# reazon-research/ReazonSpeech

Hardware: AMD Instinct MI355X
Metric: RTFx (audio-sec/wall-sec), FastConformer-RNNT 619M batch=256 (higher is better)
Workload: dtype bf16

## Files before the change

reazonspeech_amd/csrc/k_rnnt.hip:

```cpp
#include <cstdio>
#include <cstdlib>

#include "k_rnnt_common.h"

namespace {

__global__ void rnnt_init_kernel(DecodeState st, const int32_t* __restrict__ enc_lens, int B, int blank,
                                 int32_t* __restrict__ n_ids) {
    __shared__ int n_alive_s;
    if (threadIdx.x == 0) n_alive_s = 0;
    __syncthreads();
    for (int b = threadIdx.x; b < B; b += blockDim.x) {
        st.tcur[b] = 0; st.sym[b] = 0; st.token[b] = blank; st.act[b] = b;
        if (st.token2) st.token2[b] = -1;
        n_ids[b] = 0;
        if (enc_lens[b] > 0) st.alive[atomicAdd(&n_alive_s, 1)] = b;
    }
    __syncthreads();
    if (threadIdx.x == 0) { st.counters[0] = B; st.counters[1] = 0; st.counters[2] = n_alive_s; st.counters[3] = 0; }
}

__global__ __launch_bounds__(1024) void rnnt_lstm_kernel(DecodeState st, int layer, int B, int H,
                                                        const float* __restrict__ embed,
                                                        const float* __restrict__ W ,
// ... 215 lines not shown
        if (nblk >= 2) { compute(f0); f0 = f1; }
        compute(f0);
    }
#pragma unroll
    for (int ri = 0; ri < 2; ++ri)
#pragma unroll
        for (int cj = 0; cj < 4; ++cj)
#pragma unroll
            for (int r = 0; r < 4; ++r) part[wave][ri * 16 + 4 * kk + r][cj * 16 + li] = acc[ri][cj][r];
    __syncthreads();
    if (tid >= 256) { if (WALK) { __syncthreads(); continue; } return; }
    const int i = tid >> 3, c0 = (tid & 7) * 8;
    const bool row_ok = rt * 32 + i < n_rows;
    const int brow = rows_s[i];
    float best = -INFINITY;
    int best_idx = 0x7fffffff;
#pragma unroll
    for (int e = 0; e < 8; ++e) {
        const int v = ct * 64 + c0 + e;
        float s = part[0][i][c0 + e];
#pragma unroll
        for (int sl = 1; sl < SPLITK_TILE; ++sl) s = s + part[sl][i][c0 + e];
        if (v < N) {
            s = s + bias[v];
            if (MODE == 0) { if (row_ok) st.g[(size_t)brow * N + v] = s; }
            else if (!ARGMAX) { if (row_ok) st.zapprox[(size_t)brow * (64 * n_ctiles) + v] = s; }
            else if (s > best) { best = s; best_idx = v; }
        }
    }
    if (ARGMAX) {
#pragma unroll
        for (int off = 1; off < 8; off <<= 1) {
            const float ov = __shfl_xor(best, off, 64);
            const int oi = __shfl_xor(best_idx, off, 64);
            if (ov > best || (ov == best && oi < best_idx)) { best = ov; best_idx = oi; }
        }
        if ((tid & 7) == 0 && row_ok) {
            st.pmax[(size_t)brow * n_ctiles + ct] = best;
            st.pidx[(size_t)brow * n_ctiles + ct] = best_idx;
        }
    } else if (MODE == 0 && row_ok) {
        const int stride = gridDim.x * 64;
        for (int l = 0; l < L; ++l)
            for (int u = ct * 64 + c0; u < H; u += stride)
#pragma unroll
                for (int e = 0; e < 8; ++e) {
                    if (u + e >= H) break;
                    const size_t o = ((size_t)l * B + brow) * H + u + e;
                    st.h[o] = st.h_tmp[o];
                    st.c[o] = st.c_tmp[o];
                }
    }
    if (!WALK) return;
    __syncthreads();
    }
}

__global__ __launch_bounds__(256) void rnnt_finalize_kernel(DecodeState st, const int32_t* __restrict__ enc_lens,
                                                            int B, int n_ctiles, int blank, int max_symbols,
                                                            int u_max, int step, int32_t* __restrict__ ids,
                                                            int32_t* __restrict__ frames, int32_t* __restrict__ n_ids) {
    const int lane = threadIdx.x & 63;
    const int slot = blockIdx.x * 4 + (threadIdx.x >> 6);
    const int n_alive = st.counters[2 + (step & 1)];
    if (slot >= n_alive) return;
    const int b = st.alive[(size_t)(step & 1) * B + slot];
    float val = -INFINITY;
    int idx = 0x7fffffff;
    for (int ctile = lane; ctile < n_ctiles; ctile += 64) {
        const float ov = st.pmax[(size_t)b * n_ctiles + ctile];
        const int oi = st.pidx[(size_t)b * n_ctiles + ctile];
        if (ov > val || (ov == val && oi < idx)) { val = ov; idx = oi; }
    }
#pragma unroll
    for (int off = 32; off > 0; off >>= 1) {
        const float ov = __shfl_xor(val, off, 64);
        const int oi = __shfl_xor(idx, off, 64);
        if (ov > val || (ov == val && oi < idx)) { val = ov; idx = oi; }
    }
    if (lane != 0) return;
    int t = st.tcur[b], sy = st.sym[b];
    bool emitted = false;
    if (idx == blank || idx == st.unk || idx == 0x7fffffff) {
        t += 1; sy = 0;
    } else {
        const int n = n_ids[b];
        if (n < u_max) { ids[(size_t)b * u_max + n] = idx; frames[(size_t)b * u_max + n] = t; n_ids[b] = n + 1; }
        else st.counters[1] = 1;
        if (st.token2) st.token2[b] = st.token[b];
        st.token[b] = idx;
        emitted = true;
        sy += 1;
        if (sy >= max_symbols) { t += 1; sy = 0; }
    }
    st.tcur[b] = t; st.sym[b] = sy;
    if (t < enc_lens[b]) {
        const int pos = atomicAdd(&st.counters[2 + ((step + 1) & 1)], 1);
        st.alive[(size_t)((step + 1) & 1) * B + pos] = b;
        if (emitted) { const int pa = atomicAdd(&st.counters[0], 1); st.act[pa] = b; }
    }
}



__global__ __launch_bounds__(256) void rnnt_finalize_la_kernel(DecodeState st, const int32_t* __restrict__ enc_lens, int B, int n_ctiles,
                                                               int blank, int max_symbols, int u_max, int step, int la,
                                                               int32_t* __restrict__ ids, int32_t* __restrict__ frames,
                                                               int32_t* __restrict__ n_ids) {
    const int lane = threadIdx.x & 63;
    const int slot = blockIdx.x * 4 + (threadIdx.x >> 6);
    const int n_alive = st.counters[2 + (step & 1)];
    if (slot >= n_alive) return;
    const int b = st.alive[(size_t)(step & 1) * B + slot];
    const int T = enc_lens[b];
    int t = st.tcur[b], sy = st.sym[b];
    bool emitted = false;
    for (int j = 0; j < la && t < T; ++j) {
        float val = -INFINITY;
        int idx = 0x7fffffff;
        const size_t row = (size_t)b * la + j;
        for (int ctile = lane; ctile < n_ctiles; ctile += 64) {
            const float ov = st.pmax[row * n_ctiles + ctile];
            const int oi = st.pidx[row * n_ctiles + ctile];
            if (ov > val || (ov == val && oi < idx)) { val = ov; idx = oi; }
        }
#pragma unroll
        for (int off = 32; off > 0; off >>= 1) {
            const float ov = __shfl_xor(val, off, 64);
            const int oi = __shfl_xor(idx, off, 64);
            if (ov > val || (ov == val && oi < idx)) { val = ov; idx = oi; }
        }
        if (idx == blank || idx == st.unk || idx == 0x7fffffff) { t += 1; sy = 0; continue; }
        if (lane == 0) {
            const int n = n_ids[b];
            if (n < u_max) { ids[(size_t)b * u_max + n] = idx; frames[(size_t)b * u_max + n] = t; n_ids[b] = n + 1; }
            else st.counters[1] = 1;
            if (st.token2) st.token2[b] = st.token[b];
            st.token[b] = idx;
        }
        emitted = true;
        sy += 1;
        if (sy >= max_symbols) { t += 1; sy = 0; }
        break;
    }
    if (lane != 0) return;
    st.tcur[b] = t; st.sym[b] = sy;
    if (t < T) {
        const int pos = atomicAdd(&st.counters[2 + ((step + 1) & 1)], 1);
        st.alive[(size_t)((step + 1) & 1) * B + pos] = b;
        if (emitted) { const int pa = atomicAdd(&st.counters[0], 1); st.act[pa] = b; }
    }
}

__global__ __launch_bounds__(1024) void rnnt_lstm4_kernel(DecodeState st, int layer, int B, int H,
                                                         const float* __restrict__ embed,
                                                         const float* __restrict__ W4 ,
                                                         const float* __restrict__ bias ) {
    __shared__ float part[SPLITK_LSTM][32][17];
    __shared__ int rows_s[32];
    const int n_act = st.counters[0];
    const int rt = blockIdx.y, ug = blockIdx.x;
    if (rt * 32 >= n_act) return;
    const int tid = threadIdx.x, lane = tid & 63, wave = tid >> 6;
    if (tid < 32) {
        const int i = rt * 32 + tid;
        rows_s[tid] = st.act[i < n_act ? i : n_act - 1];
    }
    __syncthreads();
    const int li = lane & 15, kk = lane >> 4;
    const int lr = lane >> 2, lc = lane & 3;
    const int perm = 4 * (4 * li + kk);
    const int K = 2 * H, kslice = K / SPLITK_LSTM, nkb = K / 16;
    const float* xsrc[2];
    const float* hsrc[2];
#pragma unroll
    for (int ri = 0; ri < 2; ++ri) {
        const int row = rows_s[ri * 16 + lr];
        xsrc[ri] = layer == 0 ? embed + (size_t)st.token[row] * H : st.h_tmp + ((size_t)(layer - 1) * B + row) * H;
        hsrc[ri] = st.h + ((size_t)layer * B + row) * H;
    }
    const float* wfrag = W4 + ((size_t)ug * nkb) * 256 + lane * 4;
    f32x4_t acc[2] = {(f32x4_t){0.f, 0.f, 0.f, 0.f}, (f32x4_t){0.f, 0.f, 0.f, 0.f}};
    const int kbeg = wave * kslice, nblk = kslice / 16;
    float4 av[2][8], wv[8];
#pragma unroll
    for (int u = 0; u < 8; ++u)
        if (u < nblk) {
            const int k = kbeg + 16 * u + 4 * lc;
#pragma unroll
            for (int ri = 0; ri < 2; ++ri)
                av[ri][u] = (k < H) ? *reinterpret_cast<const float4*>(xsrc[ri] + k) : *reinterpret_cast<const float4*>(hsrc[ri] + (k - H));
            wv[u] = *reinterpret_cast<const float4*>(wfrag + (size_t)((kbeg >> 4) + u) * 256);
        }
#pragma unroll
    for (int u = 0; u < 8; ++u)
        if (u < nblk) {
            const float4 a0 = to_mfma_a_layout(av[0][u], perm), a1 = to_mfma_a_layout(av[1][u], perm);
#define RS_MFMA_E(c)                                                                         \
            acc[0] = __builtin_amdgcn_mfma_f32_16x16x4f32(a0.c, wv[u].c, acc[0], 0, 0, 0);   \
            acc[1] = __builtin_amdgcn_mfma_f32_16x16x4f32(a1.c, wv[u].c, acc[1], 0, 0, 0);
            RS_MFMA_E(x) RS_MFMA_E(y) RS_MFMA_E(z) RS_MFMA_E(w)
#undef RS_MFMA_E
        }
#pragma unroll
    for (int ri = 0; ri < 2; ++ri)
#pragma unroll
        for (int r = 0; r < 4; ++r) part[wave][ri * 16 + 4 * kk + r][li] = acc[ri][r];
    __syncthreads();
    if (tid >= 128) return;
    const int i = tid >> 2, u4 = tid & 3;
    if (rt * 32 + i >= n_act) return;
    const int brow = rows_s[i];
    const int unit = ug * 4 + u4;
    float z[4];
#pragma unroll
    for (int gt = 0; gt < 4; ++gt) {
        float sm = part[0][i][gt * 4 + u4];
#pragma unroll
        for (int sl = 1; sl < SPLITK_LSTM; ++sl) sm = sm + part[sl][i][gt * 4 + u4];
        z[gt] = sm + bias[gt * H + unit];
    }
    const float ig = rs_sigmoidf(z[0]), fg = rs_sigmoidf(z[1]), gg = rs_tanhf(z[2]), og = rs_sigmoidf(z[3]);
    const size_t o = ((size_t)layer * B + brow) * H + unit;
    const float cn = fmaf(fg, st.c[o], ig * gg);
    st.c_tmp[o] = cn;
    st.h_tmp[o] = og * rs_tanhf(cn);
}

__global__ __launch_bounds__(512) void rnnt_pred16_kernel(DecodeState st, int B, int L, int H, int N ,
                                                         const float* __restrict__ W, const float* __restrict__ bias) {
    __shared__ float part[SPLITK_TILE][32][17];
    __shared__ int rows_s[32];
    const int rt = blockIdx.y, ct = blockIdx.x;
    const int tid = threadIdx.x, lane = tid & 63, wave = tid >> 6;
    const int n_rows = st.counters[0];
    if (rt * 32 >= n_rows) return;
    if (tid < 32) {
        const int i = rt * 32 + tid;
        rows_s[tid] = st.act[i < n_rows ? i : n_rows - 1];
    }
    __syncthreads();
    const int li = lane & 15, kk = lane >> 4;
    const int lr = lane >> 2, lc = lane & 3;
    const int perm = 4 * (4 * li + kk);
    const int K = H, nkb = K / 16;
    const float* asrc[2];
#pragma unroll
    for (int ri = 0; ri < 2; ++ri) asrc[ri] = st.h_tmp + ((size_t)(L - 1) * B + rows_s[ri * 16 + lr]) * H;
    const float* wfrag = W + ((size_t)ct * nkb) * 256 + lane * 4;
    f32x4_t acc[2] = {(f32x4_t){0.f, 0.f, 0.f, 0.f}, (f32x4_t){0.f, 0.f, 0.f, 0.f}};
    const int kslice = K / SPLITK_TILE, kbeg = wave * kslice, nblk = kslice / 16;
    float4 av[2][8], wv[8];
#pragma unroll
    for (int u = 0; u < 8; ++u)
        if (u < nblk) {
            const int k = kbeg + 16 * u + 4 * lc;
#pragma unroll
            for (int ri = 0; ri < 2; ++ri) av[ri][u] = *reinterpret_cast<const float4*>(asrc[ri] + k);
            wv[u] = *reinterpret_cast<const float4*>(wfrag + (size_t)((kbeg >> 4) + u) * 256);
        }
#pragma unroll
    for (int u = 0; u < 8; ++u)
        if (u < nblk) {
            const float4 a0 = to_mfma_a_layout(av[0][u], perm), a1 = to_mfma_a_layout(av[1][u], perm);
#define RS_MFMA_E(c)                                                                         \
            acc[0] = __builtin_amdgcn_mfma_f32_16x16x4f32(a0.c, wv[u].c, acc[0], 0, 0, 0);   \
            acc[1] = __builtin_amdgcn_mfma_f32_16x16x4f32(a1.c, wv[u].c, acc[1], 0, 0, 0);
            RS_MFMA_E(x) RS_MFMA_E(y) RS_MFMA_E(z) RS_MFMA_E(w)
#undef RS_MFMA_E
        }
#pragma unroll
    for (int ri = 0; ri < 2; ++ri)
#pragma unroll
        for (int r = 0; r < 4; ++r) part[wave][ri * 16 + 4 * kk + r][li] = acc[ri][r];
    __syncthreads();
    const int i = tid >> 4, c = tid & 15;
    const bool row_ok = rt * 32 + i < n_rows;
    const int brow = rows_s[i];
    const int v = ct * 16 + c;
    if (row_ok && v < N) {
        float sm = part[0][i][c];
#pragma unroll
        for (int sl = 1; sl < SPLITK_TILE; ++sl) sm = sm + part[sl][i][c];
        st.g[(size_t)brow * N + v] = sm + bias[v];
    }
    if (row_ok) {
        const int nct = gridDim.x;
        for (int l = 0; l < L; ++l)
            for (int u = ct * 16 + c; u < H; u += nct * 16) {
                const size_t o = ((size_t)l * B + brow) * H + u;
                st.h[o] = st.h_tmp[o];
                st.c[o] = st.c_tmp[o];
            }
    }
}

__global__ __launch_bounds__(256) void rnnt_prep_kernel(DecodeState st, const float* __restrict__ f, int B, int Tp, int J,
                                                        int step) {
    const int lane = threadIdx.x & 63;
    const int slot = blockIdx.x * 4 + (threadIdx.x >> 6);
    if (blockIdx.x == 0 && threadIdx.x == 0) {
        st.counters[0] = 0;
        st.counters[2 + ((step + 1) & 1)] = 0;
    }
    if (slot >= st.counters[2 + (step & 1)]) return;
    const int b = st.alive[(size_t)(step & 1) * B + slot];
    int t = st.tcur[b];
    t = t < Tp ? t : Tp - 1;
    const float* fr = f + ((size_t)b * Tp + t) * J;
    const float* gr = st.g + (size_t)b * J;
    float ss = 0.0f;
    for (int k = 4 * lane; k < J; k += 256) {
        const float4 fv = *reinterpret_cast<const float4*>(fr + k), gv = *reinterpret_cast<const float4*>(gr + k);
        float a0, a1, a2, a3;
        if (st.joint_act) {
            a0 = rs_tanhf(fv.x + gv.x); a1 = rs_tanhf(fv.y + gv.y); a2 = rs_tanhf(fv.z + gv.z); a3 = rs_tanhf(fv.w + gv.w);
        } else {
            a0 = fmaxf(fv.x + gv.x, 0.0f); a1 = fmaxf(fv.y + gv.y, 0.0f); a2 = fmaxf(fv.z + gv.z, 0.0f); a3 = fmaxf(fv.w + gv.w, 0.0f);
        }
        ss = fmaf(a0, a0, fmaf(a1, a1, fmaf(a2, a2, fmaf(a3, a3, ss))));
        *reinterpret_cast<u16x4_t*>(st.a16 + (size_t)slot * J + k) = pack_bf16x4(a0, a1, a2, a3);
    }
    ss = wave_sum(ss);
    if (lane == 0) st.anorm[slot] = sqrtf(ss) * 1.0001f;
}

__global__ __launch_bounds__(256) void rnnt_screen_kernel(DecodeState st, const float* __restrict__ f, int B, int Tp, int J,
                                                          int Vpad, const uint16_t* __restrict__ W16,
                                                          const float* __restrict__ bpad, int step) {
    extern __shared__ __attribute__((aligned(16))) char scr_smem[];
    const int ldrow = J * 2 + 16;
    const int ct = blockIdx.x, rt = blockIdx.y;
    const int tid = threadIdx.x, lane = tid & 63, wave = tid >> 6;
    const int n_alive = st.counters[2 + (step & 1)];
    if (rt * 32 >= n_alive) return;
    const int col0 = (ct * 4 + wave) * 16;
    const bool has_cols = col0 < Vpad;
    const int li = lane & 15, kc = lane >> 4;
    const int nks = J / 32;
    const uint16_t* wrow = W16 + (size_t)((has_cols ? col0 : 0) + li) * J + kc * 8;
    bf16x8_t wf[20];
#pragma unroll
    for (int q = 0; q < 20; ++q)
        if (q < nks) wf[q] = *reinterpret_cast<const bf16x8_t*>(wrow + q * 32);
    const float bv = bpad[(has_cols ? col0 : 0) + li];
    {
        const int per_row = J / 8;
        for (int idx = tid; idx < 32 * per_row; idx += 256) {
            const int r = idx / per_row, c = idx - r * per_row;
            const int i = rt * 32 + r;
            const uint4 v = *reinterpret_cast<const uint4*>(st.a16 + (size_t)(i < n_alive ? i : n_alive - 1) * J + c * 8);
            *reinterpret_cast<uint4*>(scr_smem + r * ldrow + c * 16) = v;
        }
    }
    __syncthreads();
    if (!has_cols) return;
    f32x4_t acc[2] = {(f32x4_t){0.f, 0.f, 0.f, 0.f}, (f32x4_t){0.f, 0.f, 0.f, 0.f}};
#pragma unroll
    for (int q = 0; q < 20; ++q)
        if (q < nks) {
#pragma unroll
            for (int ri = 0; ri < 2; ++ri) {
                const bf16x8_t af = *reinterpret_cast<const bf16x8_t*>(scr_smem + (ri * 16 + li) * ldrow + (q * 32 + kc * 8) * 2);
                acc[ri] = __builtin_amdgcn_mfma_f32_16x16x32_bf16(af, wf[q], acc[ri], 0, 0, 0);
            }
        }
#pragma unroll
    for (int ri = 0; ri < 2; ++ri)
#pragma unroll
        for (int r = 0; r < 4; ++r) {
            const int slot = rt * 32 + ri * 16 + 4 * kc + r;
            if (slot < n_alive) st.zapprox[(size_t)slot * Vpad + col0 + li] = acc[ri][r] + bv;
        }
}

constexpr int VER_CAP = 1024;

__device__ __forceinline__ void verify_evaluate(const int* cand_s, int n_cand, const float* a_s, const float* __restrict__ Wrm,
                                                const float* __restrict__ bo, int J, int lane, float& best, int& best_idx) {
    const int cgrp = lane >> 3, sl = lane & 7;
    const int kslice = J / SPLITK_TILE, nblk = kslice / 16;
    for (int c0 = 0; c0 < n_cand; c0 += 8) {
        const bool valid = c0 + cgrp < n_cand;
        const int cand = valid ? cand_s[c0 + cgrp] : 0;
        const float* w = Wrm + (size_t)cand * J + sl * kslice;
        const float* as = a_s + sl * kslice;
        float4 wv[8][4];
#pragma unroll
        for (int u = 0; u < 8; ++u)
            if (u < nblk) {
#pragma unroll
                for (int kk = 0; kk < 4; ++kk) wv[u][kk] = *reinterpret_cast<const float4*>(w + 16 * u + 4 * kk);
            }
        float acc = 0.0f;
#pragma unroll
        for (int u = 0; u < 8; ++u)
            if (u < nblk) {
                float4 av[4];
#pragma unroll
                for (int kk = 0; kk < 4; ++kk) av[kk] = *reinterpret_cast<const float4*>(as + 16 * u + 4 * kk);
#define RS_CHAIN_E(cc) _Pragma("unroll") for (int kk = 0; kk < 4; ++kk) acc = fmaf(av[kk].cc, wv[u][kk].cc, acc);
                RS_CHAIN_E(x) RS_CHAIN_E(y) RS_CHAIN_E(z) RS_CHAIN_E(w)
#undef RS_CHAIN_E
            }
        float sum = __shfl(acc, lane & ~7, 64);
#pragma unroll
        for (int q = 1; q < SPLITK_TILE; ++q) sum = sum + __shfl(acc, (lane & ~7) + q, 64);
        float val = valid ? sum + bo[cand] : -INFINITY;
        int idx = valid ? cand : 0x7fffffff;
#pragma unroll
        for (int off = 8; off < 64; off <<= 1) {
            const float ov = __shfl_xor(val, off, 64);
            const int oi = __shfl_xor(idx, off, 64);
            if (ov > val || (ov == val && oi < idx)) { val = ov; idx = oi; }
        }
        if (val > best || (val == best && idx < best_idx)) { best = val; best_idx = idx; }
    }
}

__device__ __forceinline__ void verify_act_row(const DecodeState& st, const float* fr, const float* gr, float* a_s, int J, int tid, int nthr) {
    for (int k = 4 * tid; k < J; k += 4 * nthr) {
        const float4 fv = *reinterpret_cast<const float4*>(fr + k), gv = *reinterpret_cast<const float4*>(gr + k);
        if (st.joint_act)
            *reinterpret_cast<float4*>(a_s + k) = make_float4(rs_tanhf(fv.x + gv.x), rs_tanhf(fv.y + gv.y), rs_tanhf(fv.z + gv.z), rs_tanhf(fv.w + gv.w));
        else
            *reinterpret_cast<float4*>(a_s + k) = make_float4(fmaxf(fv.x + gv.x, 0.0f), fmaxf(fv.y + gv.y, 0.0f),
                                                              fmaxf(fv.z + gv.z, 0.0f), fmaxf(fv.w + gv.w, 0.0f));
    }
}

__device__ __forceinline__ void verify_commit(const DecodeState& st, int b, int t, int idx, const int32_t* __restrict__ enc_lens, int B,
                                              int blank, int max_symbols, int u_max, int step, int32_t* __restrict__ ids,
                                              int32_t* __restrict__ frames, int32_t* __restrict__ n_ids) {
    int sy = st.sym[b];
    bool emitted = false;
    if (idx == blank || idx == st.unk || idx == 0x7fffffff) {
        t += 1; sy = 0;
    } else {
        const int n = n_ids[b];
        if (n < u_max) { ids[(size_t)b * u_max + n] = idx; frames[(size_t)b * u_max + n] = t; n_ids[b] = n + 1; }
        else st.counters[1] = 1;
        if (st.token2) st.token2[b] = st.token[b];
        st.token[b] = idx;
        emitted = true;
        sy += 1;
        if (sy >= max_symbols) { t += 1; sy = 0; }
    }
    st.tcur[b] = t; st.sym[b] = sy;
    if (t < enc_lens[b]) {
        const int pos = atomicAdd(&st.counters[2 + ((step + 1) & 1)], 1);
        st.alive[(size_t)((step + 1) & 1) * B + pos] = b;
        if (emitted) { const int pa = atomicAdd(&st.counters[0], 1); st.act[pa] = b; }
    }
}

template <int NCH>
__global__ __launch_bounds__(256) void rnnt_verify_kernel(DecodeState st, const float* __restrict__ f,
                                                          const int32_t* __restrict__ enc_lens, int B, int Tp, int J, int V,
                                                          int Vpad, const float* __restrict__ Wrm ,
                                                          const float* __restrict__ bo, const float* __restrict__ wmax, int blank,
                                                          int max_symbols, int u_max, int step, int32_t* __restrict__ ids,
                                                          int32_t* __restrict__ frames, int32_t* __restrict__ n_ids) {
    extern __shared__ __attribute__((aligned(16))) char ver_smem[];
    constexpr int CAND_ROWS = NCH > 0 ? NCH * 64 : VER_CAP;
    const int lane = threadIdx.x & 63, wave = threadIdx.x >> 6;
    const int slot = blockIdx.x * 4 + wave;
    const int n_alive = st.counters[2 + (step & 1)];
    if (slot >= n_alive) return;
    const int b = st.alive[(size_t)(step & 1) * B + slot];
    const float* z = st.zapprox + (size_t)slot * Vpad;
    const int nchunk = (V + 63) / 64;
    float zr[NCH > 0 ? NCH : 1];
    float m = -INFINITY;
    if constexpr (NCH > 0) {
#pragma unroll
        for (int c = 0; c < NCH; ++c) zr[c] = (c * 64 + lane < V) ? z[c * 64 + lane] : -INFINITY;
#pragma unroll
        for (int c = 0; c < NCH; ++c) m = fmaxf(m, zr[c]);
    } else {
        for (int c = 0; c < nchunk; ++c) m = fmaxf(m, (c * 64 + lane < V) ? z[c * 64 + lane] : -INFINITY);
    }
    m = wave_max(m);
    const int t = st.tcur[b];
    const int tc = t < Tp ? t : Tp - 1;
    float* a_s = reinterpret_cast<float*>(ver_smem) + wave * J;
    verify_act_row(st, f + ((size_t)b * Tp + tc) * J, st.g + (size_t)b * J, a_s, J, lane, 64);
    const float thr = m - 0.01953125f * wmax[0] * st.anorm[slot];
    int* cand_s = reinterpret_cast<int*>(ver_smem + 4 * J * 4) + wave * CAND_ROWS;
    float best = -INFINITY;
    int best_idx = 0x7fffffff;
    int n_cand = 0;
    if constexpr (NCH > 0) {
#pragma unroll
        for (int c = 0; c < NCH; ++c) {
            const bool is = zr[c] >= thr;
            const unsigned long long mask = __ballot(is);
            if (is) cand_s[n_cand + __builtin_popcountll(mask & ((1ull << lane) - 1ull))] = c * 64 + lane;
            n_cand += __builtin_popcountll(mask);
        }
        __builtin_amdgcn_fence(__ATOMIC_ACQ_REL, "wavefront");
        __builtin_amdgcn_wave_barrier();
        verify_evaluate(cand_s, n_cand, a_s, Wrm, bo, J, lane, best, best_idx);
    } else {
        for (int c = 0; c < nchunk; ++c) {
            const bool is = c * 64 + lane < V && z[c * 64 + lane] >= thr;
            const unsigned long long mask = __ballot(is);
            if (is) cand_s[n_cand + __builtin_popcountll(mask & ((1ull << lane) - 1ull))] = c * 64 + lane;
            n_cand += __builtin_popcountll(mask);
            if (n_cand + 64 > VER_CAP || c == nchunk - 1) {
                __builtin_amdgcn_fence(__ATOMIC_ACQ_REL, "wavefront");
                __builtin_amdgcn_wave_barrier();
                verify_evaluate(cand_s, n_cand, a_s, Wrm, bo, J, lane, best, best_idx);
                __builtin_amdgcn_fence(__ATOMIC_ACQ_REL, "wavefront");
                __builtin_amdgcn_wave_barrier();
                n_cand = 0;
            }
        }
    }
    if (lane != 0) return;
    verify_commit(st, b, t, best_idx, enc_lens, B, blank, max_symbols, u_max, step, ids, frames, n_ids);
}

template <int NCHW>
__global__ __launch_bounds__(256) void rnnt_verify_wide_kernel(DecodeState st, const float* __restrict__ f,
                                                               const int32_t* __restrict__ enc_lens, int B, int Tp, int J, int V,
                                                               int Vpad, const float* __restrict__ Wrm ,
                                                               const float* __restrict__ bo, const float* __restrict__ wmax, int blank,
                                                               int max_symbols, int u_max, int step, int32_t* __restrict__ ids,
                                                               int32_t* __restrict__ frames, int32_t* __restrict__ n_ids) {
    extern __shared__ __attribute__((aligned(16))) char ver_smem[];
    const int lane = threadIdx.x & 63, wave = threadIdx.x >> 6;
    const int slot = blockIdx.x;
    const int n_alive = st.counters[2 + (step & 1)];
    if (slot >= n_alive) return;
    const int b = st.alive[(size_t)(step & 1) * B + slot];
    const float* z = st.zapprox + (size_t)slot * Vpad;
    float zr[NCHW];
#pragma unroll
    for (int c = 0; c < NCHW; ++c) {
        const int col = (wave * NCHW + c) * 64 + lane;
        zr[c] = col < V ? z[col] : -INFINITY;
    }
    float m = -INFINITY;
#pragma unroll
    for (int c = 0; c < NCHW; ++c) m = fmaxf(m, zr[c]);
    m = wave_max(m);
    float* a_s = reinterpret_cast<float*>(ver_smem);
    int* cand_s = reinterpret_cast<int*>(ver_smem + (size_t)J * 4) + wave * (NCHW * 64);
    float* red = reinterpret_cast<float*>(ver_smem + (size_t)J * 4 + (size_t)4 * NCHW * 64 * 4);
    const int t = st.tcur[b];
    const int tc = t < Tp ? t : Tp - 1;
    verify_act_row(st, f + ((size_t)b * Tp + tc) * J, st.g + (size_t)b * J, a_s, J, threadIdx.x, 256);
    if (lane == 0) red[wave] = m;
    __syncthreads();
    m = fmaxf(fmaxf(red[0], red[1]), fmaxf(red[2], red[3]));
    const float thr = m - 0.01953125f * wmax[0] * st.anorm[slot];
    int n_cand = 0;
#pragma unroll
    for (int c = 0; c < NCHW; ++c) {
        const bool is = zr[c] >= thr;
        const unsigned long long mask = __ballot(is);
        if (is) cand_s[n_cand + __builtin_popcountll(mask & ((1ull << lane) - 1ull))] = (wave * NCHW + c) * 64 + lane;
        n_cand += __builtin_popcountll(mask);
    }
    __builtin_amdgcn_fence(__ATOMIC_ACQ_REL, "wavefront");
    __builtin_amdgcn_wave_barrier();
    float best = -INFINITY;
    int best_idx = 0x7fffffff;
    verify_evaluate(cand_s, n_cand, a_s, Wrm, bo, J, lane, best, best_idx);
    if (lane == 0) { red[4 + wave] = best; reinterpret_cast<int*>(red)[8 + wave] = best_idx; }
    __syncthreads();
    if (threadIdx.x != 0) return;
#pragma unroll
    for (int w = 0; w < 4; ++w) {
        const float v = red[4 + w];
        const int i = reinterpret_cast<int*>(red)[8 + w];
        if (v > best || (v == best && i < best_idx)) { best = v; best_idx = i; }
    }
    verify_commit(st, b, t, best_idx, enc_lens, B, blank, max_symbols, u_max, step, ids, frames, n_ids);
}

}


namespace {

__global__ __launch_bounds__(256) void k2_decoder_kernel(DecodeState st, int B, int D, const float* __restrict__ embed,
                                                         const float* __restrict__ conv_w ) {
    const int n_rows = st.counters[0];
    if ((int)blockIdx.x >= n_rows) return;
    const int row = st.act[blockIdx.x];
    const int t0 = st.token2[row], t1 = st.token[row];
    for (int c = threadIdx.x; c < D; c += 256) {
        const int g4 = c & ~3;
        float acc = 0.0f;
#pragma unroll
        for (int i = 0; i < 4; ++i) {
            const float e = t0 >= 0 ? embed[(size_t)t0 * D + g4 + i] : 0.0f;
            acc = fmaf(conv_w[(c * 4 + i) * 2 + 0], e, acc);
        }
#pragma unroll
        for (int i = 0; i < 4; ++i) {
            const float e = t1 >= 0 ? embed[(size_t)t1 * D + g4 + i] : 0.0f;
            acc = fmaf(conv_w[(c * 4 + i) * 2 + 1], e, acc);
        }
        st.h_tmp[(size_t)row * D + c] = fmaxf(acc, 0.0f);
    }
}

constexpr int LSTM_LDS = SPLITK_LSTM * 4 * 32 * 16 * 4 + 32 * 4;
constexpr int TILE_LDS = SPLITK_TILE * 32 * 65 * 4 + 32 * 4;

bool narrow_kernels_usable(const rs_ctx* ctx) {
    const int L = ctx->d.pred_layers, H = ctx->d.pred_hidden;
    bool narrow = ctx->decode_narrow;
    for (int l = 0; l < L; ++l) narrow = narrow && ctx->lstm_w4[l] != nullptr;
    return narrow && 2 * H / SPLITK_LSTM / 16 <= 8 && H / SPLITK_TILE / 16 <= 8;
}

void launch_lstm_pred(rs_ctx* ctx, const DecodeState& st, int B, int rows_bound, bool narrow, hipStream_t s) {
    const int L = ctx->d.pred_layers, H = ctx->d.pred_hidden, J = ctx->d.joint_hidden;
    const int rts = (rows_bound + 31) / 32 > 0 ? (rows_bound + 31) / 32 : 1;
    if (ctx->k2_conv_w) {
        hipLaunchKernelGGL(k2_decoder_kernel, dim3(rows_bound > 0 ? rows_bound : 1), dim3(256), 0, s, st, B, H, ctx->embed, ctx->k2_conv_w);
        hipLaunchKernelGGL(rnnt_pred16_kernel, dim3((J + 15) / 16, rts), dim3(512), 0, s, st, B, 1, H, J, ctx->jpred_w, ctx->jpred_b);
        return;
    }
    if (narrow) {
        for (int l = 0; l < L; ++l)
            hipLaunchKernelGGL(rnnt_lstm4_kernel, dim3(H / 4, rts), dim3(1024), 0, s, st, l, B, H, ctx->embed, ctx->lstm_w4[l],
                               ctx->lstm_b[l]);
        hipLaunchKernelGGL(rnnt_pred16_kernel, dim3((J + 15) / 16, rts), dim3(512), 0, s, st, B, L, H, J, ctx->jpred_w,
                           ctx->jpred_b);
        return;
    }
    for (int l = 0; l < L; ++l)
        hipLaunchKernelGGL(rnnt_lstm_kernel, dim3(H / 16, rts), dim3(1024), LSTM_LDS, s, st, l, B, H, ctx->embed,
                           ctx->lstm_w[l], ctx->lstm_b[l]);
    hipLaunchKernelGGL(rnnt_tile_kernel<0>, dim3((J + 63) / 64, rts), dim3(512), TILE_LDS, s, st, (const float*)nullptr, B,
                       0, L, H, H, J, ctx->jpred_w, ctx->jpred_b, 0, 0, 1);
}

int joint_grid_x(int nct, int rts) {
    static const bool off = getenv("RS_DECODE_NO_XCD") != nullptr;
    return rts > 1 && !off ? (nct + 7) / 8 * 8 : nct;
}

int ensure_decode_lds(rs_ctx* ctx) {
    if (int rc = rs_ensure_dynamic_lds(ctx, (const void*)rnnt_lstm_kernel, LSTM_LDS); rc != RS_OK) return rc;
    if (int rc = rs_ensure_dynamic_lds(ctx, (const void*)rnnt_tile_kernel<0>, TILE_LDS); rc != RS_OK) return rc;
    if (int rc = rs_ensure_dynamic_lds(ctx, (const void*)rnnt_tile_kernel<1>, TILE_LDS); rc != RS_OK) return rc;
    if (int rc = rs_ensure_dynamic_lds(ctx, (const void*)rnnt_tile_kernel<2>, TILE_LDS); rc != RS_OK) return rc;
    if (int rc = rs_ensure_dynamic_lds(ctx, (const void*)rnnt_tile_kernel<3>, TILE_LDS); rc != RS_OK) return rc;
    if (int rc = rs_ensure_dynamic_lds(ctx, (const void*)rnnt_tile_kernel<4>, TILE_LDS); rc != RS_OK) return rc;
    return rs_ensure_dynamic_lds(ctx, (const void*)rnnt_tile_kernel<5>, TILE_LDS);
}

}

int rs_rnnt_launch_lstm_pred(rs_ctx* ctx, const void* st_ptr, int rows, hipStream_t s) {
    if (int rc = ensure_decode_lds(ctx); rc != RS_OK) return rc;
    launch_lstm_pred(ctx, *reinterpret_cast<const DecodeState*>(st_ptr), rows, rows, narrow_kernels_usable(ctx), s);
    return RS_OK;
}

int rs_rnnt_launch_joint_logits(rs_ctx* ctx, const void* st_ptr, const float* joint_enc, int rows, int tp_max, int rows_per_utt,
                                int step, hipStream_t s) {
    if (int rc = ensure_decode_lds(ctx); rc != RS_OK) return rc;
    const rs_dims& d = ctx->d;
    const int nct = (d.n_logits + 63) / 64;
    hipLaunchKernelGGL(rnnt_tile_kernel<2>, dim3(joint_grid_x(nct, (rows + 31) / 32), (rows + 31) / 32), dim3(512), TILE_LDS, s,
                       *reinterpret_cast<const DecodeState*>(st_ptr), joint_enc, rows, tp_max, d.pred_layers, d.pred_hidden,
                       d.joint_hidden, d.n_logits, ctx->jout_w, ctx->jout_b, nct, step, rows_per_utt);
    return RS_OK;
}

int rs_rnnt_launch_joint_logits_indirect(rs_ctx* ctx, const void* st_ptr, const float* joint_enc, int rows, int rows_bound, int tp_max,
                                         int rows_per_utt, int step, hipStream_t s) {
    if (int rc = ensure_decode_lds(ctx); rc != RS_OK) return rc;
    const rs_dims& d = ctx->d;
    const int nct = (d.n_logits + 63) / 64;
    const int rts = (rows_bound + 31) / 32 > 0 ? (rows_bound + 31) / 32 : 1;
    const DecodeState& st = *reinterpret_cast<const DecodeState*>(st_ptr);
    if (st.a_pre)
        hipLaunchKernelGGL(rnnt_tile_kernel<4>, dim3(joint_grid_x(nct, rts), rts), dim3(512), TILE_LDS, s, st, joint_enc, rows, tp_max,
                           d.pred_layers, d.pred_hidden, d.joint_hidden, d.n_logits, ctx->jout_w, ctx->jout_b, nct, step, rows_per_utt);
    else
        hipLaunchKernelGGL(rnnt_tile_kernel<3>, dim3(joint_grid_x(nct, rts), rts), dim3(512), TILE_LDS, s, st, joint_enc, rows, tp_max,
                           d.pred_layers, d.pred_hidden, d.joint_hidden, d.n_logits, ctx->jout_w, ctx->jout_b, nct, step, rows_per_utt);
    return RS_OK;
}

constexpr int LOOKAHEAD_MAX = 8;

static void greedy_layout(const rs_ctx* ctx, int B, rs_arena& a, DecodeState& st) {
    const rs_dims& d = ctx->d;
    const size_t state = (size_t)d.pred_layers * B * d.pred_hidden, J = d.joint_hidden;
    const size_t nct = (d.n_logits + 63) / 64, Vpad = (size_t)(d.n_logits + 15) / 16 * 16;
    st.h = a.take<float>(state); st.c = a.take<float>(state);
    st.h_tmp = a.take<float>(state); st.c_tmp = a.take<float>(state);
    st.g = a.take<float>(B * J);
    st.tcur = a.take<int32_t>(B); st.sym = a.take<int32_t>(B);
    st.token = a.take<int32_t>(B); st.act = a.take<int32_t>(B);
    if (ctx->k2_conv_w) st.token2 = a.take<int32_t>(B);
    st.alive = a.take<int32_t>((size_t)2 * B);
    st.counters = a.take<int32_t>(16);
    st.pmax = a.take<float>(B * LOOKAHEAD_MAX * nct); st.pidx = a.take<int32_t>(B * LOOKAHEAD_MAX * nct);
    st.a16 = a.take<uint16_t>(B * J); st.anorm = a.take<float>(B);
    st.zapprox = a.take<float>(B * Vpad);
}
constexpr size_t GREEDY_SLACK = 1024;

size_t rs_rnnt_workspace_bytes(const rs_ctx* ctx, int B) {
    rs_arena a;
    DecodeState st{};
    greedy_layout(ctx, B, a, st);
    return a.bytes() + GREEDY_SLACK;
}

int rs_rnnt_greedy_impl(rs_ctx* ctx, const float* joint_enc, const int32_t* enc_lens, int B, int tp_max, int u_max,
                        int32_t* ids, int32_t* frames, int32_t* n_ids, void* workspace, size_t workspace_bytes,
                        hipStream_t s) {
    const rs_dims& d = ctx->d;
    const int L = d.pred_layers, H = d.pred_hidden, J = d.joint_hidden, V = d.n_logits;
    if (B <= 0) return RS_OK;
    if (H % 128 || J % 128) return rs_fail(ctx, RS_EINVAL, "rnnt: pred_hidden/joint_hidden must be multiples of 128");
    if (L < 1 || L > 4) return rs_fail(ctx, RS_EINVAL, "rnnt: 1..4 LSTM layers supported");
    rs_arena arena(workspace);
    DecodeState st{};
    greedy_layout(ctx, B, arena, st);
    if (workspace_bytes < arena.bytes() + GREEDY_SLACK) return rs_fail(ctx, RS_EWORKSPACE, "rnnt: workspace too small");
    st.joint_act = d.joint_act;
    if (ctx->k2_conv_w) st.unk = ctx->k2 ? rs_k2_unk_id(ctx) : -1;
    const size_t state_bytes = (size_t)L * B * H * 4;
    const int nct = (V + 63) / 64, Vpad = (V + 15) / 16 * 16;
    const bool screen = ctx->decode_screen && ctx->jout_w16 && ctx->jout_wrm && ctx->jout_bpad && ctx->jout_wmax &&
                        J / SPLITK_TILE / 16 <= 8 && J / 32 <= 20;

    if (int rc = ensure_decode_lds(ctx); rc != RS_OK) return rc;
    const bool narrow = narrow_kernels_usable(ctx);
    auto lstm_and_pred = [&](int rows_bound) { launch_lstm_pred(ctx, st, B, rows_bound, narrow, s); };

    rs_prof_begin(ctx, RS_PROF_DECODE, s, 0.0, 0.0);
    RS_HIP(ctx, hipMemsetAsync(st.h, 0, 2 * rs_align(state_bytes), s));
    RS_HIP(ctx, hipMemsetAsync(st.g, 0, (size_t)B * J * 4, s));
    hipLaunchKernelGGL(rnnt_init_kernel, dim3(1), dim3(256), 0, s, st, enc_lens, B, d.blank_id, n_ids);
    lstm_and_pred(B);
    RS_CHECK_LAUNCH(ctx, "rnnt init");

    const int max_steps = tp_max + (u_max < tp_max * d.max_symbols ? u_max : tp_max * d.max_symbols) + 1;
    const int CHUNK = 16;
    const bool lookahead = getenv("RS_DECODE_NO_LOOKAHEAD") == nullptr;
    const bool verify_wide = getenv("RS_VERIFY_WIDE") && atoi(getenv("RS_VERIFY_WIDE")) != 0;
    int32_t host_counters[4] = {0, 0, 0, 0};
    int steps = 0, alive_bound = B;
    bool finished = false;
    while (!finished && steps < max_steps) {
        for (int c = 0; c < CHUNK; ++c, ++steps) {
            const int rows = alive_bound < B ? alive_bound : B;
            if (screen) {
                const int rts = (rows + 31) / 32 > 0 ? (rows + 31) / 32 : 1;
                hipLaunchKernelGGL(rnnt_prep_kernel, dim3((rows + 3) / 4 > 0 ? (rows + 3) / 4 : 1), dim3(256), 0, s, st, joint_enc, B,
                                   tp_max, J, steps);
                hipLaunchKernelGGL(rnnt_screen_kernel, dim3((Vpad + 63) / 64, rts), dim3(256), 32 * (J * 2 + 16), s, st, joint_enc, B,
                                   tp_max, J, Vpad, ctx->jout_w16, ctx->jout_bpad, steps);
                const dim3 vg((rows + 3) / 4 > 0 ? (rows + 3) / 4 : 1), vgw(rows > 0 ? rows : 1);
#define RS_VERIFY_ARGS st, joint_enc, enc_lens, B, tp_max, J, V, Vpad, ctx->jout_wrm, ctx->jout_b, ctx->jout_wmax, d.blank_id, d.max_symbols, u_max, steps, ids, frames, n_ids
                if (V > 64 * 48 && V <= 4 * 64 * 48)
                    hipLaunchKernelGGL(rnnt_verify_wide_kernel<48>, vgw, dim3(256), J * 4 + 4 * 48 * 64 * 4 + 64, s, RS_VERIFY_ARGS);
                else if (V > 64 * 48)
                    hipLaunchKernelGGL(rnnt_verify_kernel<0>, vg, dim3(256), 4 * J * 4 + 4 * VER_CAP * 4, s, RS_VERIFY_ARGS);
                else if (verify_wide)
                    hipLaunchKernelGGL(rnnt_verify_wide_kernel<12>, vgw, dim3(256), J * 4 + 4 * 12 * 64 * 4 + 64, s, RS_VERIFY_ARGS);
                else if (V <= 64 * 8)
                    hipLaunchKernelGGL(rnnt_verify_kernel<8>, vg, dim3(256), 4 * J * 4 + 4 * 8 * 64 * 4, s, RS_VERIFY_ARGS);
                else
                    hipLaunchKernelGGL(rnnt_verify_kernel<48>, vg, dim3(256), 4 * J * 4 + 4 * 48 * 64 * 4, s, RS_VERIFY_ARGS);
#undef RS_VERIFY_ARGS
            } else {
                int la = 1;
                if (lookahead) while (la < LOOKAHEAD_MAX && 2 * la * (rows > 0 ? rows : 1) <= 256) la *= 2;
                if (la > 1) {
                    const int rts = (rows * la + 31) / 32 > 0 ? (rows * la + 31) / 32 : 1;
                    hipLaunchKernelGGL(rnnt_tile_kernel<5>, dim3(joint_grid_x(nct, rts), rts), dim3(512), TILE_LDS, s, st, joint_enc, B, tp_max, L, H,
                                       J, V, ctx->jout_w, ctx->jout_b, nct, steps, la);
                    hipLaunchKernelGGL(rnnt_finalize_la_kernel, dim3((rows + 3) / 4 > 0 ? (rows + 3) / 4 : 1), dim3(256), 0, s, st, enc_lens, B, nct,
                                       d.blank_id, d.max_symbols, u_max, steps, la, ids, frames, n_ids);
                } else {
                    const int rts = (rows + 31) / 32 > 0 ? (rows + 31) / 32 : 1;
                    hipLaunchKernelGGL(rnnt_tile_kernel<1>, dim3(joint_grid_x(nct, rts), rts), dim3(512), TILE_LDS, s, st, joint_enc, B, tp_max, L, H,
                                       J, V, ctx->jout_w, ctx->jout_b, nct, steps, 1);
                    hipLaunchKernelGGL(rnnt_finalize_kernel, dim3((rows + 3) / 4 > 0 ? (rows + 3) / 4 : 1), dim3(256), 0, s, st, enc_lens, B, nct,
                                       d.blank_id, d.max_symbols, u_max, steps, ids, frames, n_ids);
                }
            }
            lstm_and_pred(rows);
        }
        RS_CHECK_LAUNCH(ctx, "rnnt step");
        RS_HIP(ctx, hipMemcpyAsync(host_counters, st.counters, 4 * sizeof(int32_t), hipMemcpyDeviceToHost, s));
        RS_HIP(ctx, hipStreamSynchronize(s));
        finished = host_counters[2 + (steps & 1)] == 0;
        alive_bound = host_counters[2 + (steps & 1)];
    }
    rs_prof_end(ctx, RS_PROF_DECODE, s);
    if (getenv("RS_DECODE_TRACE")) fprintf(stderr, "[decode trace] B=%d T'=%d: %d steps (screen %d, narrow %d, lookahead %d)\n", B, tp_max, steps, (int)screen, (int)narrow, (int)lookahead);
    if (host_counters[1]) return rs_fail(ctx, RS_EOVERFLOW, "rnnt: an utterance emitted more than u_max=%d tokens", u_max);
    if (!finished) return rs_fail(ctx, RS_ESTATE, "rnnt: decode did not finish in %d steps", max_steps);
    return RS_OK;
}
```

Before: 46460.

## Make decode LSTM/pred kernels persistent over row tiles with register-resident weights

```diff
diff --git a/reazonspeech_amd/csrc/k_rnnt.hip b/reazonspeech_amd/csrc/k_rnnt.hip
--- a/reazonspeech_amd/csrc/k_rnnt.hip
+++ b/reazonspeech_amd/csrc/k_rnnt.hip
@@ -391,49 +391,53 @@
     }
 }
 
+template <int NBLK>
 __global__ __launch_bounds__(1024) void rnnt_lstm4_kernel(DecodeState st, int layer, int B, int H,
                                                          const float* __restrict__ embed,
                                                          const float* __restrict__ W4 ,
                                                          const float* __restrict__ bias ) {
     __shared__ float part[SPLITK_LSTM][32][17];
-    __shared__ int rows_s[32];
+    __shared__ int rows_s[2][32];
     const int n_act = st.counters[0];
-    const int rt = blockIdx.y, ug = blockIdx.x;
+    int rt = blockIdx.y;
+    const int ug = blockIdx.x;
     if (rt * 32 >= n_act) return;
     const int tid = threadIdx.x, lane = tid & 63, wave = tid >> 6;
-    if (tid < 32) {
-        const int i = rt * 32 + tid;
-        rows_s[tid] = st.act[i < n_act ? i : n_act - 1];
-    }
-    __syncthreads();
     const int li = lane & 15, kk = lane >> 4;
     const int lr = lane >> 2, lc = lane & 3;
     const int perm = 4 * (4 * li + kk);
-    const int K = 2 * H, kslice = K / SPLITK_LSTM, nkb = K / 16;
-    const float* xsrc[2];
-    const float* hsrc[2];
-#pragma unroll
-    for (int ri = 0; ri < 2; ++ri) {
-        const int row = rows_s[ri * 16 + lr];
-        xsrc[ri] = layer == 0 ? embed + (size_t)st.token[row] * H : st.h_tmp + ((size_t)(layer - 1) * B + row) * H;
-        hsrc[ri] = st.h + ((size_t)layer * B + row) * H;
-    }
+    constexpr int kslice = 16 * NBLK, nkb = SPLITK_LSTM * NBLK;
+    const int kbeg = wave * kslice;
     const float* wfrag = W4 + ((size_t)ug * nkb) * 256 + lane * 4;
-    f32x4_t acc[2] = {(f32x4_t){0.f, 0.f, 0.f, 0.f}, (f32x4_t){0.f, 0.f, 0.f, 0.f}};
-    const int kbeg = wave * kslice, nblk = kslice / 16;
-    float4 av[2][8], wv[8];
-#pragma unroll
-    for (int u = 0; u < 8; ++u)
-        if (u < nblk) {
-            const int k = kbeg + 16 * u + 4 * lc;
-#pragma unroll
-            for (int ri = 0; ri < 2; ++ri)
-                av[ri][u] = (k < H) ? *reinterpret_cast<const float4*>(xsrc[ri] + k) : *reinterpret_cast<const float4*>(hsrc[ri] + (k - H));
-            wv[u] = *reinterpret_cast<const float4*>(wfrag + (size_t)((kbeg >> 4) + u) * 256);
-        }
-#pragma unroll
-    for (int u = 0; u < 8; ++u)
-        if (u < nblk) {
+    float4 wv[NBLK];
+#pragma unroll
+    for (int u = 0; u < NBLK; ++u) wv[u] = *reinterpret_cast<const float4*>(wfrag + (size_t)(wave * NBLK + u) * 256);
+    if (tid < 32) {
+        const int i = rt * 32 + tid;
+        rows_s[0][tid] = st.act[i < n_act ? i : n_act - 1];
+    }
+    __syncthreads();
+    for (int buf = 0;; buf ^= 1) {
+        const float* asrc[2];
+#pragma unroll
+        for (int ri = 0; ri < 2; ++ri) {
+            const int row = rows_s[buf][ri * 16 + lr];
+            const float* x = layer == 0 ? embed + (size_t)st.token[row] * H : st.h_tmp + ((size_t)(layer - 1) * B + row) * H;
+            asrc[ri] = (kbeg < H ? x + kbeg : st.h + ((size_t)layer * B + row) * H + (kbeg - H)) + 4 * lc;
+        }
+        f32x4_t acc[2] = {(f32x4_t){0.f, 0.f, 0.f, 0.f}, (f32x4_t){0.f, 0.f, 0.f, 0.f}};
+        float4 av[2][NBLK];
+#pragma unroll
+        for (int u = 0; u < NBLK; ++u)
+#pragma unroll
+            for (int ri = 0; ri < 2; ++ri) av[ri][u] = *reinterpret_cast<const float4*>(asrc[ri] + 16 * u);
+        const int rt_next = rt + gridDim.y;
+        if (tid < 32 && rt_next * 32 < n_act) {
+            const int i = rt_next * 32 + tid;
+            rows_s[buf ^ 1][tid] = st.act[i < n_act ? i : n_act - 1];
+        }
+#pragma unroll
+        for (int u = 0; u < NBLK; ++u) {
             const float4 a0 = to_mfma_a_layout(av[0][u], perm), a1 = to_mfma_a_layout(av[1][u], perm);
 #define RS_MFMA_E(c)                                                                         \
             acc[0] = __builtin_amdgcn_mfma_f32_16x16x4f32(a0.c, wv[u].c, acc[0], 0, 0, 0);   \
@@ -442,65 +446,75 @@
 #undef RS_MFMA_E
         }
 #pragma unroll
-    for (int ri = 0; ri < 2; ++ri)
-#pragma unroll
-        for (int r = 0; r < 4; ++r) part[wave][ri * 16 + 4 * kk + r][li] = acc[ri][r];
-    __syncthreads();
-    if (tid >= 128) return;
-    const int i = tid >> 2, u4 = tid & 3;
-    if (rt * 32 + i >= n_act) return;
-    const int brow = rows_s[i];
-    const int unit = ug * 4 + u4;
-    float z[4];
-#pragma unroll
-    for (int gt = 0; gt < 4; ++gt) {
-        float sm = part[0][i][gt * 4 + u4];
-#pragma unroll
-        for (int sl = 1; sl < SPLITK_LSTM; ++sl) sm = sm + part[sl][i][gt * 4 + u4];
-        z[gt] = sm + bias[gt * H + unit];
-    }
-    const float ig = rs_sigmoidf(z[0]), fg = rs_sigmoidf(z[1]), gg = rs_tanhf(z[2]), og = rs_sigmoidf(z[3]);
-    const size_t o = ((size_t)layer * B + brow) * H + unit;
-    const float cn = fmaf(fg, st.c[o], ig * gg);
-    st.c_tmp[o] = cn;
-    st.h_tmp[o] = og * rs_tanhf(cn);
-}
-
+        for (int ri = 0; ri < 2; ++ri)
+#pragma unroll
+            for (int r = 0; r < 4; ++r) part[wave][ri * 16 + 4 * kk + r][li] = acc[ri][r];
+        __syncthreads();
+        const int i = tid >> 2, u4 = tid & 3;
+        if (tid < 128 && rt * 32 + i < n_act) {
+            const int brow = rows_s[buf][i];
+            const int unit = ug * 4 + u4;
+            float z[4];
+#pragma unroll
+            for (int gt = 0; gt < 4; ++gt) {
+                float sm = part[0][i][gt * 4 + u4];
+#pragma unroll
+                for (int sl = 1; sl < SPLITK_LSTM; ++sl) sm = sm + part[sl][i][gt * 4 + u4];
+                z[gt] = sm + bias[gt * H + unit];
+            }
+            const float ig = rs_sigmoidf(z[0]), fg = rs_sigmoidf(z[1]), gg = rs_tanhf(z[2]), og = rs_sigmoidf(z[3]);
+            const size_t o = ((size_t)layer * B + brow) * H + unit;
+            const float cn = fmaf(fg, st.c[o], ig * gg);
+            st.c_tmp[o] = cn;
+            st.h_tmp[o] = og * rs_tanhf(cn);
+        }
+        rt = rt_next;
+        if (rt * 32 >= n_act) return;
+        __syncthreads();
+    }
+}
+
+template <int NBLK>
 __global__ __launch_bounds__(512) void rnnt_pred16_kernel(DecodeState st, int B, int L, int H, int N ,
                                                          const float* __restrict__ W, const float* __restrict__ bias) {
     __shared__ float part[SPLITK_TILE][32][17];
-    __shared__ int rows_s[32];
-    const int rt = blockIdx.y, ct = blockIdx.x;
+    __shared__ int rows_s[2][32];
+    int rt = blockIdx.y;
+    const int ct = blockIdx.x;
     const int tid = threadIdx.x, lane = tid & 63, wave = tid >> 6;
     const int n_rows = st.counters[0];
     if (rt * 32 >= n_rows) return;
-    if (tid < 32) {
-        const int i = rt * 32 + tid;
-        rows_s[tid] = st.act[i < n_rows ? i : n_rows - 1];
-    }
-    __syncthreads();
     const int li = lane & 15, kk = lane >> 4;
     const int lr = lane >> 2, lc = lane & 3;
     const int perm = 4 * (4 * li + kk);
-    const int K = H, nkb = K / 16;
-    const float* asrc[2];
-#pragma unroll
-    for (int ri = 0; ri < 2; ++ri) asrc[ri] = st.h_tmp + ((size_t)(L - 1) * B + rows_s[ri * 16 + lr]) * H;
+    constexpr int kslice = 16 * NBLK, nkb = SPLITK_TILE * NBLK;
+    const int kbeg = wave * kslice;
     const float* wfrag = W + ((size_t)ct * nkb) * 256 + lane * 4;
-    f32x4_t acc[2] = {(f32x4_t){0.f, 0.f, 0.f, 0.f}, (f32x4_t){0.f, 0.f, 0.f, 0.f}};
-    const int kslice = K / SPLITK_TILE, kbeg = wave * kslice, nblk = kslice / 16;
-    float4 av[2][8], wv[8];
-#pragma unroll
-    for (int u = 0; u < 8; ++u)
-        if (u < nblk) {
-            const int k = kbeg + 16 * u + 4 * lc;
-#pragma unroll
-            for (int ri = 0; ri < 2; ++ri) av[ri][u] = *reinterpret_cast<const float4*>(asrc[ri] + k);
-            wv[u] = *reinterpret_cast<const float4*>(wfrag + (size_t)((kbeg >> 4) + u) * 256);
-        }
-#pragma unroll
-    for (int u = 0; u < 8; ++u)
-        if (u < nblk) {
+    float4 wv[NBLK];
+#pragma unroll
+    for (int u = 0; u < NBLK; ++u) wv[u] = *reinterpret_cast<const float4*>(wfrag + (size_t)(wave * NBLK + u) * 256);
+    if (tid < 32) {
+        const int i = rt * 32 + tid;
+        rows_s[0][tid] = st.act[i < n_rows ? i : n_rows - 1];
+    }
+    __syncthreads();
+    for (int buf = 0;; buf ^= 1) {
+        const float* asrc[2];
+#pragma unroll
+        for (int ri = 0; ri < 2; ++ri) asrc[ri] = st.h_tmp + ((size_t)(L - 1) * B + rows_s[buf][ri * 16 + lr]) * H;
+        f32x4_t acc[2] = {(f32x4_t){0.f, 0.f, 0.f, 0.f}, (f32x4_t){0.f, 0.f, 0.f, 0.f}};
+        float4 av[2][NBLK];
+#pragma unroll
+        for (int u = 0; u < NBLK; ++u)
+#pragma unroll
+            for (int ri = 0; ri < 2; ++ri) av[ri][u] = *reinterpret_cast<const float4*>(asrc[ri] + kbeg + 16 * u + 4 * lc);
+        const int rt_next = rt + gridDim.y;
+        if (tid < 32 && rt_next * 32 < n_rows) {
+            const int i = rt_next * 32 + tid;
+            rows_s[buf ^ 1][tid] = st.act[i < n_rows ? i : n_rows - 1];
+        }
+#pragma unroll
+        for (int u = 0; u < NBLK; ++u) {
             const float4 a0 = to_mfma_a_layout(av[0][u], perm), a1 = to_mfma_a_layout(av[1][u], perm);
 #define RS_MFMA_E(c)                                                                         \
             acc[0] = __builtin_amdgcn_mfma_f32_16x16x4f32(a0.c, wv[u].c, acc[0], 0, 0, 0);   \
@@ -509,28 +523,32 @@
 #undef RS_MFMA_E
         }
 #pragma unroll
-    for (int ri = 0; ri < 2; ++ri)
-#pragma unroll
-        for (int r = 0; r < 4; ++r) part[wave][ri * 16 + 4 * kk + r][li] = acc[ri][r];
-    __syncthreads();
-    const int i = tid >> 4, c = tid & 15;
-    const bool row_ok = rt * 32 + i < n_rows;
-    const int brow = rows_s[i];
-    const int v = ct * 16 + c;
-    if (row_ok && v < N) {
-        float sm = part[0][i][c];
-#pragma unroll
-        for (int sl = 1; sl < SPLITK_TILE; ++sl) sm = sm + part[sl][i][c];
-        st.g[(size_t)brow * N + v] = sm + bias[v];
-    }
-    if (row_ok) {
-        const int nct = gridDim.x;
-        for (int l = 0; l < L; ++l)
-            for (int u = ct * 16 + c; u < H; u += nct * 16) {
-                const size_t o = ((size_t)l * B + brow) * H + u;
-                st.h[o] = st.h_tmp[o];
-                st.c[o] = st.c_tmp[o];
-            }
+        for (int ri = 0; ri < 2; ++ri)
+#pragma unroll
+            for (int r = 0; r < 4; ++r) part[wave][ri * 16 + 4 * kk + r][li] = acc[ri][r];
+        __syncthreads();
+        const int i = tid >> 4, c = tid & 15;
+        const bool row_ok = rt * 32 + i < n_rows;
+        const int brow = rows_s[buf][i];
+        const int v = ct * 16 + c;
+        if (row_ok && v < N) {
+            float sm = part[0][i][c];
+#pragma unroll
+            for (int sl = 1; sl < SPLITK_TILE; ++sl) sm = sm + part[sl][i][c];
+            st.g[(size_t)brow * N + v] = sm + bias[v];
+        }
+        if (row_ok) {
+            const int nct = gridDim.x;
+            for (int l = 0; l < L; ++l)
+                for (int u = ct * 16 + c; u < H; u += nct * 16) {
+                    const size_t o = ((size_t)l * B + brow) * H + u;
+                    st.h[o] = st.h_tmp[o];
+                    st.c[o] = st.c_tmp[o];
+                }
+        }
+        rt = rt_next;
+        if (rt * 32 >= n_rows) return;
+        __syncthreads();
     }
 }
 
@@ -824,26 +842,28 @@
 
 namespace {
 
+constexpr int K2_DECODER_WGS = 64;
 __global__ __launch_bounds__(256) void k2_decoder_kernel(DecodeState st, int B, int D, const float* __restrict__ embed,
                                                          const float* __restrict__ conv_w ) {
     const int n_rows = st.counters[0];
-    if ((int)blockIdx.x >= n_rows) return;
-    const int row = st.act[blockIdx.x];
-    const int t0 = st.token2[row], t1 = st.token[row];
-    for (int c = threadIdx.x; c < D; c += 256) {
-        const int g4 = c & ~3;
-        float acc = 0.0f;
-#pragma unroll
-        for (int i = 0; i < 4; ++i) {
-            const float e = t0 >= 0 ? embed[(size_t)t0 * D + g4 + i] : 0.0f;
-            acc = fmaf(conv_w[(c * 4 + i) * 2 + 0], e, acc);
-        }
-#pragma unroll
-        for (int i = 0; i < 4; ++i) {
-            const float e = t1 >= 0 ? embed[(size_t)t1 * D + g4 + i] : 0.0f;
-            acc = fmaf(conv_w[(c * 4 + i) * 2 + 1], e, acc);
-        }
-        st.h_tmp[(size_t)row * D + c] = fmaxf(acc, 0.0f);
+    for (int r = blockIdx.x; r < n_rows; r += gridDim.x) {
+        const int row = st.act[r];
+        const int t0 = st.token2[row], t1 = st.token[row];
+        for (int c = threadIdx.x; c < D; c += 256) {
+            const int g4 = c & ~3;
+            float acc = 0.0f;
+#pragma unroll
+            for (int i = 0; i < 4; ++i) {
+                const float e = t0 >= 0 ? embed[(size_t)t0 * D + g4 + i] : 0.0f;
+                acc = fmaf(conv_w[(c * 4 + i) * 2 + 0], e, acc);
+            }
+#pragma unroll
+            for (int i = 0; i < 4; ++i) {
+                const float e = t1 >= 0 ? embed[(size_t)t1 * D + g4 + i] : 0.0f;
+                acc = fmaf(conv_w[(c * 4 + i) * 2 + 1], e, acc);
+            }
+            st.h_tmp[(size_t)row * D + c] = fmaxf(acc, 0.0f);
+        }
     }
 }
 
@@ -857,20 +877,33 @@
     return narrow && 2 * H / SPLITK_LSTM / 16 <= 8 && H / SPLITK_TILE / 16 <= 8;
 }
 
-void launch_lstm_pred(rs_ctx* ctx, const DecodeState& st, int B, int rows_bound, bool narrow, hipStream_t s) {
+constexpr int ACT_TILES_Y = 1;
+
+void launch_lstm_pred(rs_ctx* ctx, const DecodeState& st, int B, int rows_bound, bool narrow, bool exact_rows, hipStream_t s) {
     const int L = ctx->d.pred_layers, H = ctx->d.pred_hidden, J = ctx->d.joint_hidden;
     const int rts = (rows_bound + 31) / 32 > 0 ? (rows_bound + 31) / 32 : 1;
+    const int act_tiles_y = exact_rows || rts < ACT_TILES_Y ? rts : ACT_TILES_Y;
+#define RS_BY_NBLK(KERNEL, ...)                                                                                       \
+    switch (H / 128) {                                                                                                \
+        case 1: hipLaunchKernelGGL(KERNEL<1>, __VA_ARGS__); break; case 2: hipLaunchKernelGGL(KERNEL<2>, __VA_ARGS__); break; \
+        case 3: hipLaunchKernelGGL(KERNEL<3>, __VA_ARGS__); break; case 4: hipLaunchKernelGGL(KERNEL<4>, __VA_ARGS__); break; \
+        case 5: hipLaunchKernelGGL(KERNEL<5>, __VA_ARGS__); break; case 6: hipLaunchKernelGGL(KERNEL<6>, __VA_ARGS__); break; \
+        case 7: hipLaunchKernelGGL(KERNEL<7>, __VA_ARGS__); break; default: hipLaunchKernelGGL(KERNEL<8>, __VA_ARGS__); break; \
+    }
     if (ctx->k2_conv_w) {
-        hipLaunchKernelGGL(k2_decoder_kernel, dim3(rows_bound > 0 ? rows_bound : 1), dim3(256), 0, s, st, B, H, ctx->embed, ctx->k2_conv_w);
-        hipLaunchKernelGGL(rnnt_pred16_kernel, dim3((J + 15) / 16, rts), dim3(512), 0, s, st, B, 1, H, J, ctx->jpred_w, ctx->jpred_b);
+        const int rows = rows_bound > 0 ? rows_bound : 1;
+        const int wgs = exact_rows || rows < K2_DECODER_WGS ? rows : K2_DECODER_WGS;
+        hipLaunchKernelGGL(k2_decoder_kernel, dim3(wgs), dim3(256), 0, s, st, B, H, ctx->embed, ctx->k2_conv_w);
+        RS_BY_NBLK(rnnt_pred16_kernel, dim3((J + 15) / 16, act_tiles_y), dim3(512), 0, s, st, B, 1, H, J, ctx->jpred_w,
+                   ctx->jpred_b);
         return;
     }
     if (narrow) {
         for (int l = 0; l < L; ++l)
-            hipLaunchKernelGGL(rnnt_lstm4_kernel, dim3(H / 4, rts), dim3(1024), 0, s, st, l, B, H, ctx->embed, ctx->lstm_w4[l],
-                               ctx->lstm_b[l]);
-        hipLaunchKernelGGL(rnnt_pred16_kernel, dim3((J + 15) / 16, rts), dim3(512), 0, s, st, B, L, H, J, ctx->jpred_w,
-                           ctx->jpred_b);
+            RS_BY_NBLK(rnnt_lstm4_kernel, dim3(H / 4, act_tiles_y), dim3(1024), 0, s, st, l, B, H, ctx->embed, ctx->lstm_w4[l],
+                       ctx->lstm_b[l]);
+        RS_BY_NBLK(rnnt_pred16_kernel, dim3((J + 15) / 16, act_tiles_y), dim3(512), 0, s, st, B, L, H, J, ctx->jpred_w,
+                   ctx->jpred_b);
         return;
     }
     for (int l = 0; l < L; ++l)
@@ -878,6 +911,7 @@
                            ctx->lstm_w[l], ctx->lstm_b[l]);
     hipLaunchKernelGGL(rnnt_tile_kernel<0>, dim3((J + 63) / 64, rts), dim3(512), TILE_LDS, s, st, (const float*)nullptr, B,
                        0, L, H, H, J, ctx->jpred_w, ctx->jpred_b, 0, 0, 1);
+#undef RS_BY_NBLK
 }
 
 int joint_grid_x(int nct, int rts) {
@@ -899,7 +933,7 @@
 
 int rs_rnnt_launch_lstm_pred(rs_ctx* ctx, const void* st_ptr, int rows, hipStream_t s) {
     if (int rc = ensure_decode_lds(ctx); rc != RS_OK) return rc;
-    launch_lstm_pred(ctx, *reinterpret_cast<const DecodeState*>(st_ptr), rows, rows, narrow_kernels_usable(ctx), s);
+    launch_lstm_pred(ctx, *reinterpret_cast<const DecodeState*>(st_ptr), rows, rows, narrow_kernels_usable(ctx), true, s);
     return RS_OK;
 }
 
@@ -978,7 +1012,7 @@
 
     if (int rc = ensure_decode_lds(ctx); rc != RS_OK) return rc;
     const bool narrow = narrow_kernels_usable(ctx);
-    auto lstm_and_pred = [&](int rows_bound) { launch_lstm_pred(ctx, st, B, rows_bound, narrow, s); };
+    auto lstm_and_pred = [&](int rows_bound) { launch_lstm_pred(ctx, st, B, rows_bound, narrow, false, s); };
 
     rs_prof_begin(ctx, RS_PROF_DECODE, s, 0.0, 0.0);
     RS_HIP(ctx, hipMemsetAsync(st.h, 0, 2 * rs_align(state_bytes), s));
```

New measurement: 46440 (median of 2 runs). Within noise of the previous version (-0.0%).
